# StoreyLab/terastructure

Hardware: AMD Instinct MI355X
Metric: SNP-minibatch updates/sec (N x K phi+accum) at N=1000000 K=8 (higher is better)
Workload: dtype f64

## Files before the change

### terastructure_amd/csrc/tsamd_hybrid_kernels.h

```cpp
#pragma once
#include "tsamd_resident_kernels.h"

namespace tsamd {


template <int KT>
__device__ __forceinline__ void hy_gamma_one(double (&gx)[KT], double (&wx)[KT], uint32_t nib, uint32_t &cn, const double *s_sb, const DevParams &p) {
  const double mom = (double)(nib & 3u), dad = (double)((nib >> 2) & 3u);
  const bool ok = (nib & 15u) != 0u;
  double s0 = 0.0, s1 = 0.0;
  uint32_t zo = 0u;
  asm volatile("" : "+v"(zo));
  const double *sbv = s_sb + zo;
#pragma unroll
  for (int k = 0; k < KT; ++k) {
    s0 = fma(wx[k], sbv[2 * k], s0);
    s1 = fma(wx[k], sbv[2 * k + 1], s1);
  }
  const double rho = ok ? fast_rsqrt(p.nodetau0 + (double)cn) : 0.0;
  const double inv = fast_rcp(s0 * s1) * (rho * p.gamma_scale);
  const double c0 = (mom * s1) * inv, c1 = (dad * s0) * inv, keep = 1.0 - rho, ra = rho * p.alpha;
#pragma unroll
  for (int k = 0; k < KT; ++k) gx[k] = fma(wx[k], fma(c0, sbv[2 * k], c1 * sbv[2 * k + 1]), fma(keep, gx[k], ra));
  if constexpr (KT <= 8) gamma_to_w<KT>(gx, wx); else gamma_to_w_lean<KT>(gx, wx);
  cn = ok ? cn + 1u : cn;
}

template <int KT, int WR, bool STREAM>
__global__ __launch_bounds__(256, 1) void ts_hybrid(Ctl *ctl_a, double *w_a, uint32_t npad_a, uint32_t chunk_a, uint32_t par_arg,
                                                    const uint32_t *sched, uint32_t n_sched, ResXchg *xb, uint32_t serial, const DevParams p) {
  constexpr int BLOCK = 256, kWaves = BLOCK / 64, R = hy_reg_items(KT), Q = hy_lds_items(KT), RQ = R + Q;
  constexpr bool BS = KT <= 12, BSC = KT <= 8;
  constexpr uint32_t J = 2 * KT;
  static_assert(resident_vec(KT) == 1 && R <= 16 && Q >= 1 && Q <= 16, "one individual per item; an item class's codes share one register");
  __shared__ __attribute__((aligned(16))) double s_eb[J];
  __shared__ __attribute__((aligned(16))) double s_sb[J];
  __shared__ double s_lam[J], s_diff[J], s_tot[res_tot_doubles<KT, WR>()], s_plam[J], s_peb[J];
  __shared__ double s_red[kWaves * J];
  __shared__ int s_alive[4];
  __shared__ double s_w[Q][KT][BLOCK];
  const uint32_t par = par_arg & 1u;
  Ctl *ctl = ctl_a;
  const State *S = &ctl->st[par ^ 1u];
  State *W = &ctl->st[par];
  const uint32_t svalid = S->valid, sloc = S->loc, shol = S->hol, siters = S->iters, sidx = S->idx;
  const unsigned long long epoch_now = S->epoch + 1ull;
  const uint32_t xseq0 = ctl->xseq;
  uint32_t tid = threadIdx.x;
  const size_t np = npad_a;
  const uint32_t nitems = npad_a;
  const uint32_t begin = blockIdx.x * chunk_a, end = min(begin + chunk_a, nitems);
  uint32_t i0 = begin + tid;
  uint32_t cnt = (i0 < end) ? (end - i0 + BLOCK - 1u) / BLOCK : 0u;
  auto fresh = [&]() { asm volatile("" : "+v"(tid), "+v"(i0), "+v"(cnt)); };
  auto item_or_last = [&](uint32_t t) { return min(i0, nitems - 1u) + min(t, max(cnt, 1u) - 1u) * BLOCK; };
  const uint32_t cnt_wg = begin < end ? (end - begin + BLOCK - 1u) / BLOCK : 0u;
  const uint32_t scnt_wg = (STREAM && cnt_wg > (uint32_t)RQ) ? cnt_wg - (uint32_t)RQ : 0u;
  const uint32_t g = blockIdx.x % (uint32_t)kResGroups, m = blockIdx.x / (uint32_t)kResGroups;

  if (__hip_atomic_load(&xb->abort_word, __ATOMIC_RELAXED, __HIP_MEMORY_SCOPE_AGENT) != 0ull) return;
  if (n_sched == 0u) {
    if (blockIdx.x == 0) carry_state(S, W, J);
    return;
  }
  if (tid < 4) s_alive[tid] = 1;
  __syncthreads();
  uint32_t xcount = 1u;
  if (!res_exchange<KT, WR>(xb, p, xseq0 + 1u, 1u, 0.0, g, m, gridDim.x, s_tot, s_alive, tid, fail_code(xseq0 + 1u, true, par, serial),
                            WR == 0 ? (unsigned long long)p.probe_ticks : kResWaitTicks))
    return;
  if constexpr (WR > 0) {
    xcount += 1u;
    if (!res_exchange<KT, WR>(xb, p, xseq0 + xcount, 1u, 0.0, g, m, gridDim.x, s_tot, s_alive, tid, fail_code(xseq0 + xcount, true, par, serial),
                              kResWaitTicks / 3ull))
      return;
  }
  double buf[R][KT];
#pragma unroll
  for (int t = 0; t < R; ++t) {
#pragma unroll
    for (int k = 0; k < KT; ++k) buf[t][k] = (w_a + (size_t)k * np)[item_or_last((uint32_t)t)];
    if (t & 1) __builtin_amdgcn_sched_barrier(0);
  }
#pragma unroll
  for (int q = 0; q < Q; ++q) {
    const uint32_t i = item_or_last((uint32_t)(R + q));
#pragma unroll
    for (int k = 0; k < KT; ++k) s_w[q][k][tid] = (w_a + (size_t)k * np)[i];
  }
  auto load_codes = [&](uint32_t loc_, auto first_c, auto n_c) -> uint2 {
    constexpr int FIRST = decltype(first_c)::value, N = decltype(n_c)::value;
    const uint32_t *col = reinterpret_cast<const uint32_t *>(p.bed + (size_t)loc_ * p.colstride);
    uint32_t word[N];
#pragma unroll
    for (int t = 0; t < N; ++t) word[t] = col[item_or_last((uint32_t)(FIRST + t)) / 16u];
    uint32_t out[2] = {0u, 0u};
#pragma unroll
    for (int t = 0; t < N; ++t) {
      const uint32_t i = item_or_last((uint32_t)(FIRST + t));
      const uint32_t c = (uint32_t)(FIRST + t) < cnt ? (word[t] >> (2u * (i % 16u))) & 3u : 1u;
      out[t / 8] |= code_nibble(c) << (4u * (uint32_t)(t % 8));
    }
    return make_uint2(out[0], out[1]);
  };
  using IC0 = std::integral_constant<int, 0>;
  using ICR = std::integral_constant<int, R>;
  using ICQ = std::integral_constant<int, Q>;
  uint2 pcodes = svalid ? load_codes(sloc, IC0{}, ICR{}) : make_uint2(0u, 0u), pcodes2 = svalid ? load_codes(sloc, ICR{}, ICQ{}) : make_uint2(0u, 0u);
  if (tid < J) {
    s_sb[tid] = S->eb[tid];
    s_plam[tid] = svalid ? p.lam[(size_t)sloc * J + tid] : 0.0;
    s_peb[tid] = svalid ? p.eb[(size_t)sloc * J + tid] : 0.0;
  }
  bool do_gamma = svalid != 0u && shol == 0u;
  bool prev_valid = svalid != 0u;
  uint32_t prev_loc = sloc, prev_hol = shol, prev_iters = siters;
  bool w_dirty = false;
  unsigned long long tp_run = ctl->total_passes;
  uint32_t last_it = ctl->last_iters;
  auto count_snp_deferred = [&](uint32_t its) {
    const uint32_t bin = min(its, (uint32_t)TSAMD_PASS_HIST_BINS - 1u);
    __hip_atomic_fetch_add(&ctl->pass_hist[bin], 1ull, __ATOMIC_RELAXED, __HIP_MEMORY_SCOPE_AGENT);
    tp_run += (unsigned long long)its;
    last_it = its;
  };
#ifdef TSAMD_SCHED_TIME
  unsigned long long tk_gamma = 0, tk_sweep = 0, tk_xchg = 0, tk_epi = 0, tk_fold = 0, tk_mark = wall_clock64();
  const unsigned long long tk_start = tk_mark;
#define TSAMD_HK(acc)                               \
  do {                                              \
    const unsigned long long now_ = wall_clock64(); \
    acc += now_ - tk_mark;                          \
    tk_mark = now_;                                 \
  } while (0)
#else
#define TSAMD_HK(acc) \
  do {                \
  } while (0)
#endif
  __syncthreads();

  uint32_t iters = 0u;
  double lam_old = 0.0, eb_used = 0.0;
  double b0[BS ? KT : 1], b1[BS ? KT : 1], acc0[KT], acc1[KT];
  bool complete = false;
  uint2 codes = make_uint2(0u, 0u), codes2 = make_uint2(0u, 0u);
  uint32_t loc = 0u, hol = 0u;
  const uint32_t *col = nullptr;

  auto begin_pass = [&]() {
    fresh();
    iters += 1u;
    lam_old = s_lam[tid < J ? tid : 0u];
    eb_used = s_eb[tid < J ? tid : 0u];
#pragma unroll
    for (int k = 0; k < KT; ++k) {
      if constexpr (BSC) {
        b0[k] = uniform_f64(s_eb[2 * k]);
        b1[k] = uniform_f64(s_eb[2 * k + 1]);
      } else if constexpr (BS) {
        b0[k] = s_eb[2 * k];
        b1[k] = s_eb[2 * k + 1];
      }
      acc0[k] = acc1[k] = 0.0;
    }
  };
  auto consume = [&](const double (&wcur)[KT], uint32_t nib) {
    uint32_t zo = 0u;
    if constexpr (!BS) asm volatile("" : "+v"(zo));
    res_consume_md<KT, BS>(wcur, (double)(nib & 3u), (double)(nib >> 2), b0, b1, reinterpret_cast<const double2 *>(s_eb) + zo, acc0, acc1);
  };
  auto load_streamed = [&](uint32_t s, double (&wv)[KT], uint32_t &word) {
    const uint32_t i = item_or_last((uint32_t)RQ + s);
#pragma unroll
    for (int k = 0; k < KT; ++k) wv[k] = (w_a + (size_t)k * np)[i];
    word = col[i / 16u];
  };
  auto streamed_code = [&](uint32_t s, uint32_t word) -> uint32_t {
    const uint32_t i = item_or_last((uint32_t)RQ + s);
    return code_nibble((uint32_t)RQ + s < cnt ? (word >> (2u * (i % 16u))) & 3u : 1u);
  };
  double sa[KT], sbuf[KT];
  uint32_t worda = 0u, wordb = 0u;
  auto request_first = [&]() { load_streamed(0u, sa, worda); };
  auto sweep = [&]() {
#pragma unroll
    for (int t = 0; t < R; ++t) {
      if ((uint32_t)t >= cnt_wg) continue;
      fresh();
      double wcur[KT];
#pragma unroll
      for (int k = 0; k < KT; ++k) wcur[k] = buf[t][k];
      consume(wcur, nibble_of(codes, t));
      __builtin_amdgcn_sched_barrier(0);
    }
#pragma unroll
    for (int q = 0; q < Q; ++q) {
      if ((uint32_t)(R + q) >= cnt_wg) continue;
      fresh();
      double wcur[KT];
#pragma unroll
      for (int k = 0; k < KT; ++k) wcur[k] = s_w[q][k][tid];
      consume(wcur, nibble_of(codes2, q));
      __builtin_amdgcn_sched_barrier(0);
    }
    for (uint32_t s = 0; STREAM && s < scnt_wg; s += 2u) {
      fresh();
      load_streamed(s + 1u, sbuf, wordb);
      __builtin_amdgcn_sched_barrier(0);
      consume(sa, streamed_code(s, worda));
      __builtin_amdgcn_sched_barrier(0);
      if (s + 1u >= scnt_wg) break;
      fresh();
      load_streamed(s + 2u, sa, worda);
      __builtin_amdgcn_sched_barrier(0);
      consume(sbuf, streamed_code(s + 1u, wordb));
      __builtin_amdgcn_sched_barrier(0);
    }
  };
  auto finish_pass = [&]() -> bool {
    fresh();
    res_fold<KT>(acc0, acc1, s_red, tid);
    __syncthreads();
    TSAMD_HK(tk_fold);
    double mine = 0.0;
    if (tid < J) {
      mine = s_red[tid];
#pragma unroll
      for (int wv = 1; wv < kWaves; ++wv) mine += s_red[wv * J + tid];
    }
    xcount += 1u;
    const uint32_t tag = xseq0 + xcount;
    const bool ahead = STREAM && iters < p.max_inner;
    auto overlap = [&]() {
      if constexpr (STREAM)
        if (ahead) request_first();
    };
    if (!res_exchange<KT, WR, kResOneLevelGrid, ResLay<KT>>(xb, p, tag, 1u, mine, g, m, gridDim.x, s_tot, s_alive, tid, fail_code(tag, false, par, serial),
                                                            kResWaitTicks, overlap))
      return false;
    TSAMD_HK(tk_xchg);
    if (tid < J) epilogue_values(p, res_total<KT, WR>(s_tot, tid), eb_used, lam_old, s_lam, s_eb, s_diff);
    __syncthreads();
    complete = epilogue_complete(p, iters, J, s_diff);
    TSAMD_HK(tk_epi);
    return true;
  };

  for (uint32_t idx = 0; idx < n_sched; ++idx) {
    const uint32_t ent = sched[idx];
    loc = ent & 0x7fffffffu;
    hol = ent >> 31;
    fresh();
    if (tid < J) {
      const bool local = prev_valid && loc == prev_loc;
      const double gl = __hip_atomic_load(&p.lam[(size_t)loc * J + tid], __ATOMIC_RELAXED, __HIP_MEMORY_SCOPE_AGENT);
      const double ge = __hip_atomic_load(&p.eb[(size_t)loc * J + tid], __ATOMIC_RELAXED, __HIP_MEMORY_SCOPE_AGENT);
      s_lam[tid] = local ? s_plam[tid] : gl;
      s_eb[tid] = local ? s_peb[tid] : ge;
    }
    codes = load_codes(loc, IC0{}, ICR{});
    codes2 = load_codes(loc, ICR{}, ICQ{});
    iters = 0u;
    if (do_gamma) {
      const uint32_t *pcol = reinterpret_cast<const uint32_t *>(p.bed + (size_t)prev_loc * p.colstride);
      double gs[KT];
      uint32_t cs = 0u;
      auto load_gamma = [&](uint32_t i, double (&gq)[KT], uint32_t &cq) {
#pragma unroll
        for (int k = 0; k < KT; ++k) gq[k] = (p.gam + (size_t)k * np)[i];
        cq = p.cnt[i];
      };
      auto store_gamma = [&](uint32_t i, const double (&gq)[KT], uint32_t cq) {
#pragma unroll
        for (int k = 0; k < KT; ++k) (p.gam + (size_t)k * np)[i] = gq[k];
        p.cnt[i] = cq;
      };
      load_gamma(item_or_last(0u), gs, cs);
#pragma unroll
      for (int t = 0; t < RQ; ++t) {
        if ((uint32_t)t >= cnt_wg) continue;
        fresh();
        const uint32_t i = item_or_last((uint32_t)t);
        double gv[KT];
        uint32_t cv = cs;
#pragma unroll
        for (int k = 0; k < KT; ++k) gv[k] = gs[k];
        if ((uint32_t)(t + 1) < cnt_wg && t + 1 < RQ) load_gamma(item_or_last((uint32_t)t + 1u), gs, cs);
        __builtin_amdgcn_sched_barrier(0);
        double wcur[KT];
        if (t < R) {
#pragma unroll
          for (int k = 0; k < KT; ++k) wcur[k] = buf[t < R ? t : 0][k];
        } else {
#pragma unroll
          for (int k = 0; k < KT; ++k) wcur[k] = s_w[t < R ? 0 : t - R][k][tid];
        }
        const uint32_t pcode = t < R ? nibble_of(pcodes, t < R ? t : 0) : nibble_of(pcodes2, t < R ? 0 : t - R);
        hy_gamma_one<KT>(gv, wcur, pcode, cv, s_sb, p);
        if ((uint32_t)t < cnt) store_gamma(i, gv, cv);
        if (t < R) {
#pragma unroll
          for (int k = 0; k < KT; ++k) buf[t < R ? t : 0][k] = wcur[k];
        } else {
#pragma unroll
          for (int k = 0; k < KT; ++k) s_w[t < R ? 0 : t - R][k][tid] = wcur[k];
        }
        __builtin_amdgcn_sched_barrier(0);
      }
      if (STREAM && scnt_wg > 0u) {
        double wsn[KT];
        uint32_t pwn = 0u;
        auto load_sitem = [&](uint32_t s) {
          const uint32_t i = item_or_last((uint32_t)RQ + s);
          load_gamma(i, gs, cs);
#pragma unroll
          for (int k = 0; k < KT; ++k) wsn[k] = (w_a + (size_t)k * np)[i];
          pwn = pcol[i / 16u];
        };
        load_sitem(0u);
        for (uint32_t s = 0; s < scnt_wg; ++s) {
          fresh();
          const uint32_t i = item_or_last((uint32_t)RQ + s);
          double gv[KT], wcur[KT];
          uint32_t cv = cs;
          const uint32_t pw = pwn;
#pragma unroll
          for (int k = 0; k < KT; ++k) {
            gv[k] = gs[k];
            wcur[k] = wsn[k];
          }
          load_sitem(min(s + 1u, scnt_wg - 1u));
          __builtin_amdgcn_sched_barrier(0);
          const uint32_t pcode = code_nibble((uint32_t)RQ + s < cnt ? (pw >> (2u * (i % 16u))) & 3u : 1u);
          hy_gamma_one<KT>(gv, wcur, pcode, cv, s_sb, p);
          if ((uint32_t)RQ + s < cnt) {
            store_gamma(i, gv, cv);
#pragma unroll
            for (int k = 0; k < KT; ++k) (w_a + (size_t)k * np)[i] = wcur[k];
          }
          __builtin_amdgcn_sched_barrier(0);
        }
      }
      w_dirty = true;
    }
    col = reinterpret_cast<const uint32_t *>(p.bed + (size_t)loc * p.colstride);
    if constexpr (STREAM) request_first();
    __syncthreads();
    TSAMD_HK(tk_gamma);
    complete = false;
    while (!complete) {
      begin_pass();
      sweep();
      TSAMD_HK(tk_sweep);
      if (!finish_pass()) return;
    }
    const double fin_lam = s_lam[tid < J ? tid : 0u], fin_eb = s_eb[tid < J ? tid : 0u];
    if (blockIdx.x == 0) {
      if (tid < J) {
        __hip_atomic_store(&p.lam[(size_t)loc * J + tid], fin_lam, __ATOMIC_RELAXED, __HIP_MEMORY_SCOPE_AGENT);
        __hip_atomic_store(&p.eb[(size_t)loc * J + tid], fin_eb, __ATOMIC_RELAXED, __HIP_MEMORY_SCOPE_AGENT);
      }
      if (tid == 0) count_snp_deferred(iters);
      asm volatile("s_waitcnt vmcnt(0)" ::: "memory");
    }
    __syncthreads();
    if (tid < J) {
      s_sb[tid] = eb_used;
      s_plam[tid] = fin_lam;
      s_peb[tid] = fin_eb;
    }
    pcodes = codes;
    pcodes2 = codes2;
    do_gamma = hol == 0u;
    prev_valid = true;
    prev_loc = loc;
    prev_hol = hol;
    prev_iters = iters;
    __syncthreads();
  }

  if (w_dirty) {
#pragma unroll
    for (int t = 0; t < RQ; ++t) {
      fresh();
      if ((uint32_t)t < cnt) {
        const uint32_t i = i0 + (uint32_t)t * BLOCK;
#pragma unroll
        for (int k = 0; k < KT; ++k) (w_a + (size_t)k * np)[i] = t < R ? buf[t < R ? t : 0][k] : s_w[t < R ? 0 : t - R][k][tid];
      }
    }
  }
  fresh();
  if (blockIdx.x == 0) {
    if (tid < J) {
      W->lam[tid] = s_plam[tid];
      W->eb[tid] = s_sb[tid];
    }
    if (tid == 0) {
      W->idx = sidx + n_sched;
      W->valid = 1u;
      W->loc = prev_loc;
      W->hol = prev_hol;
// ... 29 lines not shown
```

### terastructure_amd/csrc/tsamd_resident_kernels.h

```cpp
#pragma once
#include <type_traits>

#include "tsamd_kernels.h"

namespace tsamd {
#ifndef TSAMD_NOCOL_K
#define TSAMD_NOCOL_K 0
#endif
#ifndef TSAMD_GAMMA_SB_READLANE
#define TSAMD_GAMMA_SB_READLANE 1
#endif
#ifndef TSAMD_REPL_READLANE
#define TSAMD_REPL_READLANE 1
#endif


constexpr int res_blocks(int k) { return (4 * k + 31) / 32; }
constexpr int kResMaxGran = 32 * res_blocks(kResidentMaxK);
constexpr int kResRegionRows = kResGroups * kResMembers + 2 * kResGroups;
constexpr int kResWideGran = 512;
struct ResXchg {
  unsigned long long abort_word;
  unsigned long long pad_[31];
  unsigned long long gran[2 * kResRegionRows * kResMaxGran];
// ... 581 lines not shown
    for (int k = 0; k < KT; ++k) wv[k] = reinterpret_cast<const WT *>(w_a + (size_t)k * np)[i];
  };
  if (tid < 4) s_alive[tid] = 1;

  RowSum<BLOCK> rowsum;
  rowsum.issue(partials_a + (size_t)(par ^ 1u) * kMaxGrid * J, nrows_hint, J);
  const PendingIn pin = load_pending(S, J);
  WT buf[kItems][KT];
  load_rows(item_or_last(0), buf[0]);
  __builtin_amdgcn_sched_barrier(0);
  uint32_t codes = 0u;
  {
    const uint32_t *col = reinterpret_cast<const uint32_t *>(p.bed + (size_t)sloc * p.colstride);
    uint32_t word[kItems];
#pragma unroll
    for (int t = 0; t < kItems; ++t) word[t] = col[item_or_last((uint32_t)t) / RC::kItemsPerWord];
#pragma unroll
    for (int t = 0; t < kItems; ++t) {
      const uint32_t i = item_or_last((uint32_t)t);
      const uint32_t c = (uint32_t)t < cnt ? (word[t] >> (RC::kCodeBits * (i % RC::kItemsPerWord))) & RC::kMask : RC::kMissing;
      codes |= c << (RC::kCodeBits * (uint32_t)t);
    }
  }
  __builtin_amdgcn_sched_barrier(0);

  if (aborted != 0ull) return;
  const bool pending = svalid != 0u && sdone == 0u;
  const unsigned long long epoch_now = S->epoch + 1ull;
  if (!pending) {
    if (blockIdx.x == 0) carry_state(S, W, J);
    return;
  }
  const double vrow = (snrows == nrows_hint) ? rowsum.finish()
                                             : row_partial_sum<BLOCK>(partials_a + (size_t)(par ^ 1u) * kMaxGrid * J, snrows, J);
  bool complete = finish_pending<BLOCK>(p, pin, vrow, J, s_fin, s_lam, s_eb, s_diff);
  uint32_t iters = siters;
  double eb_used = pin.eb_used;
  const uint32_t g = blockIdx.x % (uint32_t)kResGroups, m = blockIdx.x / (uint32_t)kResGroups;
  double lam_old = 0.0;
  double b0[BS ? KT : 1], b1[BS ? KT : 1], acc0[KT], acc1[KT];
  auto begin_pass = [&]() {
    iters += 1u;
    lam_old = s_lam[tid < J ? tid : 0u];
    eb_used = s_eb[tid < J ? tid : 0u];
#pragma unroll
    for (int k = 0; k < KT; ++k) {
      if constexpr (BSC) {
        b0[k] = uniform_f64(s_eb[2 * k]);
        b1[k] = uniform_f64(s_eb[2 * k + 1]);
      } else if constexpr (BS) {
        b0[k] = s_eb[2 * k];
        b1[k] = s_eb[2 * k + 1];
      }
      acc0[k] = acc1[k] = 0.0;
    }
  };
  auto consume = [&](int t, const WT (&wv)[KT]) {
    uint32_t zo = 0u;
    if constexpr (!BS) asm volatile("" : "+v"(zo));
    res_consume<KT, VEC, BS>(wv, (codes >> (RC::kCodeBits * (uint32_t)t)) & RC::kMask, b0, b1, reinterpret_cast<const double2 *>(s_eb) + zo, acc0,
                             acc1);
  };
  uint32_t xcount = 0u;
  auto finish_pass = [&]() -> bool {
    res_fold<KT>(acc0, acc1, s_red, tid);
    __syncthreads();
    double row = 0.0;
    if (tid < J) {
      row = s_red[tid];
#pragma unroll
      for (int wv = 1; wv < kWaves; ++wv) row += s_red[wv * J + tid];
    }
    if (iters >= p.max_inner) {
      if (tid < J) (partials_a + (size_t)par * kMaxGrid * J)[(size_t)blockIdx.x * J + tid] = row;
      if (blockIdx.x == 0) {
        if (tid < J) {
          W->lam[tid] = lam_old;
          W->eb[tid] = eb_used;
        }
        if (tid == 0) {
          W->idx = sidx;
          W->valid = 1u;
          W->loc = sloc;
          W->hol = shol;
          W->iters = iters;
          W->done = 0u;
          W->nrows = gridDim.x;
          W->epoch = epoch_now;
          ctl->xseq = xseq0 + xcount;
        }
      }
      return true;
    }
    xcount += 1u;
    const uint32_t tag = xseq0 + xcount;
    if (!res_exchange<KT, 0, (KT <= 8 ? 16 : 0)>(xb, p, tag, 1u, row, g, m, gridDim.x, s_tot, s_alive, tid, fail_code(tag, xcount == 1u, par, serial),
                             xcount == 1u ? (unsigned long long)p.probe_ticks : kResWaitTicks))
      return true;
    if (tid < J) epilogue_values(p, s_tot[tid], eb_used, lam_old, s_lam, s_eb, s_diff);
    __syncthreads();
    complete = epilogue_complete(p, iters, J, s_diff);
    return false;
  };
  auto publish = [&]() {
    if (blockIdx.x == 0) {
      publish_complete_v(p, ctl, W, J, sidx, sloc, shol, iters, epoch_now, eb_used, s_lam, s_eb);
      if (tid == 0) ctl->xseq = xseq0 + xcount;
    }
  };

  if (complete) {
    publish();
    return;
  }
  begin_pass();
  if constexpr (kItems > 1) load_rows(item_or_last(1u), buf[1]);
#pragma unroll
  for (int t = 0; t < kItems; ++t) {
    if (t + 2 < kItems) load_rows(item_or_last((uint32_t)t + 2u), buf[t + 2]);
    __builtin_amdgcn_sched_barrier(0);
    consume(t, buf[t]);
    __builtin_amdgcn_sched_barrier(0);
  }
  if (finish_pass()) return;
  for (;;) {
    if (complete) {
      publish();
      return;
    }
    begin_pass();
#pragma unroll
    for (int t = 0; t < kItems; ++t) {
      consume(t, buf[t]);
      __builtin_amdgcn_sched_barrier(0);
    }
    if (finish_pass()) return;
  }
}

constexpr int sched_lds_items(int k, int items, int vec) {
#ifdef TSAMD_SCHED_LDS_ITEMS
  return TSAMD_SCHED_LDS_ITEMS < items ? TSAMD_SCHED_LDS_ITEMS : items;
#else
  const int small = 1536 + 26 * 2 * k * 8;
  const int per_item = (k * 8 + 4) * vec * 256, n = (160 * 1024 - small) / per_item;
  return n < items ? n : items;
#endif
}
constexpr int sched_next_streamed(int t, int lds, int items) {
  for (int u = t + 1; u < items; ++u)
    if (((u + 1) * lds) / items == (u * lds) / items) return u;
  return items;
}

template <int KT, bool PARTIAL, int WR>
__global__ __launch_bounds__(256, 1) void ts_schedule(Ctl *ctl_a, double *w_a, uint32_t npad_a, uint32_t chunk_a, uint32_t par_arg,
                                                      const uint32_t *sched, uint32_t n_sched, ResXchg *xb, uint32_t serial, const DevParams p) {
  constexpr int BLOCK = 256, kWaves = BLOCK / 64, VEC = resident_vec(KT), kItems = sched_items(KT, WR);
  constexpr bool BS = KT <= 24, BSC = KT <= 8;
  using LN = Lanes<VEC>;
  using WT = typename LN::T;
  using CT = typename LN::C;
  using RC = ResCodes<VEC>;
  constexpr uint32_t J = 2 * KT;
  static_assert(VEC == 1 && kItems <= 16, "one individual per item; the items' genotype nibbles are packed into two registers");
  __shared__ __attribute__((aligned(16))) double s_eb[J];
  __shared__ __attribute__((aligned(16))) double s_sb[J];
  __shared__ double s_lam[J], s_diff[J], s_tot[res_tot_doubles<KT, WR>()], s_plam[J], s_peb[J];
  __shared__ double s_drow[J], s_dlam[J], s_dolam[J], s_doeb[J], s_ddiff[J];
#if defined(TSAMD_SHARED_EPILOGUE)
  constexpr bool kRepl = false;
#else
  constexpr bool kRepl = KT <= 8;
#endif
  __shared__ __attribute__((aligned(16))) double s_ebw[kWaves][J];
  __shared__ double s_diffw[kWaves][J];
  __shared__ double s_red[kWaves * J];
  __shared__ int s_alive[4];
  constexpr int kLds = sched_lds_items(KT, kItems, VEC);
  __shared__ WT s_gam[kLds > 0 ? kLds : 1][KT][BLOCK];
  __shared__ CT s_cn[kLds > 0 ? kLds : 1][BLOCK];
  auto is_lds = [](int t) { return ((t + 1) * kLds) / kItems != (t * kLds) / kItems; };
  auto lds_slot = [](int t) { return (t * kLds) / kItems; };
  const uint32_t par = par_arg & 1u;
  Ctl *ctl = ctl_a;
  const State *S = &ctl->st[par ^ 1u];
  State *W = &ctl->st[par];
  const uint32_t svalid = S->valid, sloc = S->loc, shol = S->hol, siters = S->iters, sidx = S->idx;
  const unsigned long long epoch_now = S->epoch + 1ull;
  const uint32_t xseq0 = ctl->xseq;
  uint32_t tid = threadIdx.x;
  const size_t np = npad_a;
  const uint32_t nitems = npad_a / (uint32_t)VEC;
  const uint32_t begin = blockIdx.x * chunk_a, end = min(begin + chunk_a, nitems);
  uint32_t i0 = begin + tid;
  uint32_t cnt = (i0 < end) ? min((end - i0 + BLOCK - 1u) / BLOCK, (uint32_t)kItems) : 0u;
  auto fresh = [&]() { asm volatile("" : "+v"(tid), "+v"(i0), "+v"(cnt)); };
  auto item_or_last = [&](uint32_t t) { return min(i0, nitems - 1u) + min(t, max(cnt, 1u) - 1u) * BLOCK; };
  const uint32_t cnt_wg = !PARTIAL ? (uint32_t)kItems : begin < end ? min((end - begin + BLOCK - 1u) / BLOCK, (uint32_t)kItems) : 0u;
  const uint32_t g = blockIdx.x % (uint32_t)kResGroups, m = blockIdx.x / (uint32_t)kResGroups;

  if (__hip_atomic_load(&xb->abort_word, __ATOMIC_RELAXED, __HIP_MEMORY_SCOPE_AGENT) != 0ull) return;
  if (n_sched == 0u) {
    if (blockIdx.x == 0) carry_state(S, W, J);
    return;
  }
  if (tid < 4) s_alive[tid] = 1;
  __syncthreads();
  uint32_t xcount = 1u;
  if (!res_exchange<KT, WR>(xb, p, xseq0 + 1u, 1u, 0.0, g, m, gridDim.x, s_tot, s_alive, tid, fail_code(xseq0 + 1u, true, par, serial),
                            WR == 0 ? (unsigned long long)p.probe_ticks : kResWaitTicks))
    return;
  if constexpr (WR > 0) {
    xcount += 1u;
    if (p.xchg_test_delay != 0u) {
      const unsigned long long t0 = wall_clock64();
      while (wall_clock64() - t0 < (unsigned long long)p.xchg_test_delay) __builtin_amdgcn_s_sleep(8);
    }
    if (!res_exchange<KT, WR>(xb, p, xseq0 + xcount, 1u, 0.0, g, m, gridDim.x, s_tot, s_alive, tid, fail_code(xseq0 + xcount, true, par, serial),
                              kResWaitTicks / 3ull))
      return;
  }
  WT buf[kItems][KT];
#pragma unroll
  for (int t = 0; t < kItems; ++t) {
#pragma unroll
    for (int k = 0; k < KT; ++k) buf[t][k] = reinterpret_cast<const WT *>(w_a + (size_t)k * np)[item_or_last((uint32_t)t)];
    if (t & 1) __builtin_amdgcn_sched_barrier(0);
  }
#pragma unroll
  for (int t = 0; t < kItems; ++t)
    if (is_lds(t)) {
      const uint32_t i = item_or_last((uint32_t)t);
#pragma unroll
      for (int k = 0; k < KT; ++k) s_gam[lds_slot(t)][k][tid] = reinterpret_cast<const WT *>(p.gam + (size_t)k * np)[i];
      s_cn[lds_slot(t)][tid] = reinterpret_cast<const CT *>(p.cnt)[i];
    }
  auto get_item = [&](int t, WT (&wv)[KT]) {
#pragma unroll
    for (int k = 0; k < KT; ++k) wv[k] = buf[t][k];
  };
  auto put_item = [&](int t, const WT (&wv)[KT]) {
#pragma unroll
    for (int k = 0; k < KT; ++k) buf[t][k] = wv[k];
  };
  auto get_lgamma = [&](int t, WT (&gv)[KT], CT &cv) {
#pragma unroll
    for (int k = 0; k < KT; ++k) gv[k] = s_gam[lds_slot(t)][k][tid];
    cv = s_cn[lds_slot(t)][tid];
  };
  auto put_lgamma = [&](int t, const WT (&gv)[KT], const CT &cv) {
#pragma unroll
    for (int k = 0; k < KT; ++k) s_gam[lds_slot(t)][k][tid] = gv[k];
    s_cn[lds_slot(t)][tid] = cv;
  };
  auto load_words = [&](uint32_t loc_, auto &word) {
    const uint32_t *col = reinterpret_cast<const uint32_t *>(p.bed + (size_t)loc_ * p.colstride);
#pragma unroll
    for (int t = 0; t < kItems; ++t) word[t] = col[item_or_last((uint32_t)t) / RC::kItemsPerWord];
  };
  auto pack_codes = [&](const auto &word) -> uint2 {
    uint32_t out[2] = {0u, 0u};
#pragma unroll
    for (int t = 0; t < kItems; ++t) {
      const uint32_t i = item_or_last((uint32_t)t);
      const uint32_t c = (uint32_t)t < cnt ? (word[t] >> (RC::kCodeBits * (i % RC::kItemsPerWord))) & RC::kMask : RC::kMissing;
      out[t / 8] |= code_nibble(c) << (4u * (uint32_t)(t % 8));
    }
    return make_uint2(out[0], out[1]);
  };
  auto load_codes = [&](uint32_t loc_) -> uint2 {
    uint32_t word[kItems];
    load_words(loc_, word);
    return pack_codes(word);
  };
  uint2 pcodes = svalid ? load_codes(sloc) : make_uint2(0u, 0u);
  const double sb_state = S->eb[(tid & 63u) < J ? (tid & 63u) : 0u];
  if (tid < J) {
    s_sb[tid] = S->eb[tid];
    s_plam[tid] = svalid ? p.lam[(size_t)sloc * J + tid] : 0.0;
    s_peb[tid] = svalid ? p.eb[(size_t)sloc * J + tid] : 0.0;
  }
  bool do_gamma = svalid != 0u && shol == 0u;
  bool prev_valid = svalid != 0u;
  uint32_t prev_loc = sloc, prev_hol = shol, prev_iters = siters;
  bool w_dirty = false;
  bool deferred = false;
  uint32_t dloc = 0u, diters = 0u;
  bool pub_pending = false;
  unsigned long long tp_run = ctl->total_passes;
  uint32_t last_it = ctl->last_iters;
  auto count_snp_deferred = [&](uint32_t its) {
    const uint32_t bin = min(its, (uint32_t)TSAMD_PASS_HIST_BINS - 1u);
    __hip_atomic_fetch_add(&ctl->pass_hist[bin], 1ull, __ATOMIC_RELAXED, __HIP_MEMORY_SCOPE_AGENT);
    tp_run += (unsigned long long)its;
    last_it = its;
  };
#ifdef TSAMD_SCHED_RAMP
  unsigned long long ramp_mark = wall_clock64();
  uint32_t ramp_idx = 0u;
#endif
#ifdef TSAMD_SCHED_TIME
  unsigned long long tk_gamma = 0, tk_first = 0, tk_rest = 0, tk_xchg = 0, tk_head = 0, tk_tail = 0, tk_mark = wall_clock64();
  unsigned long long tk_fold = 0, tk_epi = 0, tk_sweep = 0;
  const unsigned long long tk_start = tk_mark;
#define TSAMD_TK(acc)                         \
  do {                                        \
    const unsigned long long now_ = wall_clock64(); \
    acc += now_ - tk_mark;                    \
    tk_mark = now_;                           \
  } while (0)
#else
#define TSAMD_TK(acc) \
  do {                \
  } while (0)
#endif
  __syncthreads();

  uint32_t iters = 0u;
  double lam_old = 0.0, eb_used = 0.0;
  double b0[BS ? KT : 1], b1[BS ? KT : 1], acc0[KT], acc1[KT];
  bool complete = false;
  constexpr bool kColAhead = !(KT == 16 || KT == 14 || (KT == 24 && WR == 8)) && KT != TSAMD_NOCOL_K;
  uint2 codes = kColAhead ? load_codes(sched[0] & 0x7fffffffu) : make_uint2(0u, 0u);
  uint32_t nword[kColAhead ? kItems : 1];
  double eb_ran = sb_state;
  auto begin_pass = [&]() {
    fresh();
    iters += 1u;
    const double *bsrc = kRepl ? s_ebw[tid >> 6] : s_eb;
    if constexpr (kRepl) {
      eb_ran = eb_used;
    } else {
      lam_old = s_lam[tid < J ? tid : 0u];
      eb_used = s_eb[tid < J ? tid : 0u];
    }
#pragma unroll
    for (int k = 0; k < KT; ++k) {
      if constexpr (kRepl && BSC && TSAMD_REPL_READLANE) {
        b0[k] = lane_f64(eb_used, 2 * k);
        b1[k] = lane_f64(eb_used, 2 * k + 1);
      } else if constexpr (BSC) {
        b0[k] = uniform_f64(bsrc[2 * k]);
        b1[k] = uniform_f64(bsrc[2 * k + 1]);
      } else if constexpr (BS) {
        b0[k] = bsrc[2 * k];
        b1[k] = bsrc[2 * k + 1];
      }
      acc0[k] = acc1[k] = 0.0;
    }
  };
  auto sweep = [&]() {
#ifdef TSAMD_SCHED_TIME
    const unsigned long long ts0 = wall_clock64();
#endif
#pragma unroll
    for (int t = 0; t < kItems; ++t) {
      if (PARTIAL && (uint32_t)t >= cnt_wg) continue;
      fresh();
      WT wcur[KT];
      get_item(t, wcur);
      uint32_t zo = 0u;
      if constexpr (!BS) asm volatile("" : "+v"(zo));
      const double2 *bl = reinterpret_cast<const double2 *>(kRepl ? s_ebw[tid >> 6] : s_eb) + zo;
      {
        const uint32_t nib = nibble_of(codes, t);
        res_consume_md<KT, BS>(wcur, (double)(nib & 3u), (double)(nib >> 2), b0, b1, bl, acc0, acc1);
      }
      __builtin_amdgcn_sched_barrier(0);
    }
#ifdef TSAMD_SCHED_TIME
    tk_sweep += wall_clock64() - ts0;
#endif
  };
  auto finish_pass = [&](bool defer) -> bool {
    fresh();
#ifdef TSAMD_SCHED_TIME
    const unsigned long long tf0 = wall_clock64();
#endif
    if (kRepl && pub_pending) {
      asm volatile("s_waitcnt vmcnt(0)" ::: "memory");
      pub_pending = false;
    }
    res_fold<KT>(acc0, acc1, s_red, tid);
    __syncthreads();
#ifdef TSAMD_SCHED_TIME
    const unsigned long long tx0 = wall_clock64();
    tk_fold += tx0 - tf0;
#endif
    double mine = 0.0;
    if (tid < J) {
      mine = s_red[tid];
#pragma unroll
      for (int wv = 1; wv < kWaves; ++wv) mine += s_red[wv * J + tid];
    }
    if (defer) {
      if (tid < J) s_drow[tid] = mine;
      if (tid < J) s_dlam[tid] = lam_old;
      complete = true;
      return true;
    }
    const uint32_t width = deferred ? 2u : 1u;
    if (deferred && tid >= 64u && tid < 64u + J) mine = s_drow[tid - 64u];
    if (!kRepl && pub_pending) {
      asm volatile("s_waitcnt vmcnt(0)" ::: "memory");
      pub_pending = false;
    }
    xcount += 1u;
    const uint32_t tag = xseq0 + xcount;
    if (!res_exchange<KT, WR>(xb, p, tag, width, mine, g, m, gridDim.x, s_tot, s_alive, tid, fail_code(tag, false, par, serial), kResWaitTicks))
      return false;
#ifdef TSAMD_SCHED_TIME
    const unsigned long long te0 = wall_clock64();
    tk_xchg += te0 - tx0;
#endif
    if constexpr (kRepl) {
      const uint32_t lane = tid & 63u, wave = tid >> 6;
      if (lane < J) {
        double nw, ebn, df;
        epilogue_values_reg(p, lane, res_total<KT, WR>(s_tot, lane), eb_used, lam_old, nw, ebn, df);
        lam_old = nw;
        eb_used = ebn;
        if constexpr (!(BSC && TSAMD_REPL_READLANE)) s_ebw[wave][lane] = ebn;
        s_diffw[wave][lane] = df;
      }
      if (deferred) {
        if (blockIdx.x == 0) {
          if (wave == 1u && lane < J) {
            double nw, ebn, df;
            epilogue_values_reg(p, lane, res_total<KT, WR>(s_tot, J + lane), s_sb[lane], s_dlam[lane], nw, ebn, df);
            __hip_atomic_store(&p.lam[(size_t)dloc * J + lane], nw, __ATOMIC_RELAXED, __HIP_MEMORY_SCOPE_AGENT);
            __hip_atomic_store(&p.eb[(size_t)dloc * J + lane], ebn, __ATOMIC_RELAXED, __HIP_MEMORY_SCOPE_AGENT);
          }
          if (tid == 0) count_snp_deferred(diters);
          pub_pending = true;
        }
        deferred = false;
      }
      complete = epilogue_complete(p, iters, J, s_diffw[wave]);
    } else {
    if (tid < J) epilogue_values(p, res_total<KT, WR>(s_tot, tid), eb_used, lam_old, s_lam, s_eb, s_diff);
    if (deferred && blockIdx.x == 0 && tid >= 64u && tid < 64u + J)
      epilogue_values_at(p, tid - 64u, res_total<KT, WR>(s_tot, J + tid - 64u), s_sb[tid - 64u], s_dlam[tid - 64u], s_dolam, s_doeb, s_ddiff);
    __syncthreads();
    if (deferred) {
      if (blockIdx.x == 0) {
        if (tid < J) {
          __hip_atomic_store(&p.lam[(size_t)dloc * J + tid], s_dolam[tid], __ATOMIC_RELAXED, __HIP_MEMORY_SCOPE_AGENT);
          __hip_atomic_store(&p.eb[(size_t)dloc * J + tid], s_doeb[tid], __ATOMIC_RELAXED, __HIP_MEMORY_SCOPE_AGENT);
        }
        if (tid == 0) count_snp_deferred(diters);
        pub_pending = true;
      }
      deferred = false;
    }
    if constexpr (KT > 8) complete = epilogue_complete_wave<J>(p, iters, s_diff, tid & 63u); else complete = epilogue_complete(p, iters, J, s_diff);
    }
#ifdef TSAMD_SCHED_TIME
    tk_epi += wall_clock64() - te0;
#endif
    return true;
  };

  uint32_t loc = 0, hol = 0;
  uint32_t ent_n = sched[0], ent_nn = sched[min(1u, n_sched - 1u)];
  double nlam = 0.0, neb = 0.0;
  if (tid < J) {
    nlam = p.lam[(size_t)(ent_n & 0x7fffffffu) * J + tid];
    neb = p.eb[(size_t)(ent_n & 0x7fffffffu) * J + tid];
  }
  for (uint32_t idx = 0; idx < n_sched; ++idx) {
    const uint32_t ent = ent_n;
    loc = ent & 0x7fffffffu;
    hol = ent >> 31;
    ent_n = ent_nn;
    ent_nn = sched[min(idx + 2u, n_sched - 1u)];
    if (tid < J) {
      const bool local = prev_valid && loc == prev_loc;
      s_lam[tid] = local ? s_plam[tid] : nlam;
      s_eb[tid] = local ? s_peb[tid] : neb;
    }
    fresh();
    if constexpr (!kColAhead) codes = load_codes(loc);
    __syncthreads();
    if constexpr (kRepl) {
      const uint32_t lane = tid & 63u, wave = tid >> 6;
      lam_old = s_lam[lane < J ? lane : 0u];
      eb_used = s_eb[lane < J ? lane : 0u];
      if constexpr (!(BSC && TSAMD_REPL_READLANE))
        if (lane < J) s_ebw[wave][lane] = eb_used;
    }
    iters = 0u;
    TSAMD_TK(tk_head);
    if (do_gamma) {
      WT gs[KT];
      CT cs;
      auto load_gamma = [&](uint32_t i, WT (&gq)[KT], CT &cq) {
#pragma unroll
        for (int k = 0; k < KT; ++k) gq[k] = reinterpret_cast<const WT *>(p.gam + (size_t)k * np)[i];
        cq = reinterpret_cast<const CT *>(p.cnt)[i];
      };
#if defined(TSAMD_LITERAL_STEP)
      constexpr bool kLeanStep = false;
#elif defined(TSAMD_LEAN_STEP)
      constexpr bool kLeanStep = true;
#else
      constexpr bool kLeanStep = PARTIAL || KT > 8;
#endif
      constexpr bool kSbScalar = kRepl && BSC && TSAMD_GAMMA_SB_READLANE != 0;
      double sbs[kSbScalar ? J : 1];
      if constexpr (kSbScalar) {
#pragma unroll
        for (int j = 0; j < (int)J; ++j) sbs[j] = lane_f64(eb_ran, j);
      }
      auto gamma_one = [&](double (&gx)[KT], double (&wx)[KT], uint32_t nib, uint32_t &cn) {
        const double mom = (double)(nib & 3u), dad = (double)((nib >> 2) & 3u);
        const bool ok = (nib & 15u) != 0u;
        double s0 = 0.0, s1 = 0.0;
        uint32_t zo = 0u;
        asm volatile("" : "+v"(zo));
        const double *sbv = s_sb + zo;
        auto sb = [&](int j) -> double {
          if constexpr (kSbScalar) return sbs[j]; else return sbv[j];
        };
#pragma unroll
        for (int k = 0; k < KT; ++k) {
          s0 = fma(wx[k], sb(2 * k), s0);
          s1 = fma(wx[k], sb(2 * k + 1), s1);
        }
        const double rho = ok ? fast_rsqrt(p.nodetau0 + (double)cn) : 0.0;
        if constexpr (kLeanStep) {
          const double inv = fast_rcp(s0 * s1) * (rho * p.gamma_scale);
          const double c0 = (mom * s1) * inv, c1 = (dad * s0) * inv, keep = 1.0 - rho, ra = rho * p.alpha;
#pragma unroll
          for (int k = 0; k < KT; ++k) gx[k] = fma(wx[k], fma(c0, sb(2 * k), c1 * sb(2 * k + 1)), fma(keep, gx[k], ra));
        } else {
          const double c0 = mom * fast_rcp(s0), c1 = dad * fast_rcp(s1);
#pragma unroll
          for (int k = 0; k < KT; ++k) {
            const double e = c0 * (wx[k] * sb(2 * k)) + c1 * (wx[k] * sb(2 * k + 1));
            gx[k] += rho * (p.alpha + p.gamma_scale * e - gx[k]);
          }
        }
        if constexpr (KT <= 8) gamma_to_w<KT>(gx, wx); else gamma_to_w_lean<KT>(gx, wx);
        cn = ok ? cn + 1u : cn;
      };
      constexpr int kFirstStreamed = sched_next_streamed(-1, kLds, kItems);
      if (kFirstStreamed < kItems) load_gamma(item_or_last((uint32_t)kFirstStreamed), gs, cs);
#pragma unroll
      for (int t = 0; t < kItems; ++t) {
        if (PARTIAL && (uint32_t)t >= cnt_wg) continue;
        fresh();
        const uint32_t i = item_or_last((uint32_t)t);
        const bool mine = (uint32_t)t < cnt;
        WT gv[KT];
        CT cv;
        if (is_lds(t)) {
          get_lgamma(t, gv, cv);
        } else {
#pragma unroll
          for (int k = 0; k < KT; ++k) gv[k] = gs[k];
          cv = cs;
          constexpr int kNone = kItems;
          const int nxt = sched_next_streamed(t, kLds, kItems);
          if (nxt < kNone) load_gamma(item_or_last((uint32_t)nxt), gs, cs);
        }
        __builtin_amdgcn_sched_barrier(0);
        WT wcur[KT];
        get_item(t, wcur);
        uint32_t pcode = nibble_of(pcodes, t);
        if constexpr (VEC == 2) {
#pragma unroll 1
          for (int v = 0; v < 2; ++v) {
            double gx[KT], wx[KT];
#pragma unroll
            for (int k = 0; k < KT; ++k) {
              gx[k] = gv[k].x;
              wx[k] = wcur[k].x;
            }
            uint32_t cn = cv.x;
            gamma_one(gx, wx, pcode, cn);
            pcode >>= 2;
            cv.x = cv.y;
            cv.y = cn;
#pragma unroll
            for (int k = 0; k < KT; ++k) {
              gv[k].x = gv[k].y;
              gv[k].y = gx[k];
              wcur[k].x = wcur[k].y;
              wcur[k].y = wx[k];
            }
          }
        } else {
          gamma_one(gv, wcur, pcode, cv);
        }
        if (is_lds(t)) {
          put_lgamma(t, gv, cv);
        } else if (mine) {
#pragma unroll
          for (int k = 0; k < KT; ++k) reinterpret_cast<WT *>(p.gam + (size_t)k * np)[i] = gv[k];
          reinterpret_cast<CT *>(p.cnt)[i] = cv;
        }
        put_item(t, wcur);
        __builtin_amdgcn_sched_barrier(0);
      }
      w_dirty = true;
    }
    TSAMD_TK(tk_gamma);
    begin_pass();
    sweep();
    if (!finish_pass(false)) return;
    TSAMD_TK(tk_first);
    fresh();
    if (tid < J) {
      nlam = __hip_atomic_load(&p.lam[(size_t)(ent_n & 0x7fffffffu) * J + tid], __ATOMIC_RELAXED, __HIP_MEMORY_SCOPE_AGENT);
      neb = __hip_atomic_load(&p.eb[(size_t)(ent_n & 0x7fffffffu) * J + tid], __ATOMIC_RELAXED, __HIP_MEMORY_SCOPE_AGENT);
    }
    if constexpr (kColAhead) load_words(ent_n & 0x7fffffffu, nword);
    while (!complete) {
      begin_pass();
      sweep();
#ifdef TSAMD_NO_DEFER
      const bool defer = false;
#else
      const bool defer = iters >= p.max_inner && idx + 1u < n_sched && (ent_n & 0x7fffffffu) != loc &&
                         (idx + 2u >= n_sched || (ent_nn & 0x7fffffffu) != loc);
#endif
      if (!finish_pass(defer)) return;
      if (defer) {
        deferred = true;
        dloc = loc;
        diters = iters;
      }
    }
    TSAMD_TK(tk_rest);
    const double fin_lam = kRepl ? lam_old : s_lam[tid < J ? tid : 0u], fin_eb = kRepl ? eb_used : s_eb[tid < J ? tid : 0u];
    if (!deferred && blockIdx.x == 0) {
      if (tid < J) {
        __hip_atomic_store(&p.lam[(size_t)loc * J + tid], fin_lam, __ATOMIC_RELAXED, __HIP_MEMORY_SCOPE_AGENT);
        __hip_atomic_store(&p.eb[(size_t)loc * J + tid], fin_eb, __ATOMIC_RELAXED, __HIP_MEMORY_SCOPE_AGENT);
      }
      if (tid == 0) count_snp_deferred(iters);
      asm volatile("s_waitcnt vmcnt(0)" ::: "memory");
    }
    __syncthreads();
    if (tid < J) s_sb[tid] = kRepl ? eb_ran : eb_used;
    if (tid < J) {
      s_plam[tid] = fin_lam;
      s_peb[tid] = fin_eb;
    }
    pcodes = codes;
    fresh();
    if constexpr (kColAhead) codes = pack_codes(nword);
    do_gamma = hol == 0u;
    prev_valid = true;
    prev_loc = loc;
    prev_hol = hol;
    prev_iters = iters;
    __syncthreads();
    TSAMD_TK(tk_tail);
#ifdef TSAMD_SCHED_RAMP
    if (blockIdx.x == 0 && tid == 0) {
      const uint32_t marks[8] = {5u, 20u, 50u, 100u, 200u, 500u, 1000u, 2000u};
      for (int q = 0; q < 8; ++q)
        if (idx + 1u == marks[q]) {
          const unsigned long long now = wall_clock64();
          printf("ts_schedule ramp: SNPs up to %u: %.2f us per SNP in this range (launch of %u)\n", marks[q],
                 (now - ramp_mark) * 0.01 / (double)(marks[q] - ramp_idx), n_sched);
          ramp_mark = now;
          ramp_idx = marks[q];
        }
    }
#endif
  }

  if (w_dirty) {
#pragma unroll
    for (int t = 0; t < kItems; ++t) {
      fresh();
      if ((uint32_t)t < cnt) {
        const uint32_t i = i0 + (uint32_t)t * BLOCK;
        WT wcur[KT];
        get_item(t, wcur);
#pragma unroll
        for (int k = 0; k < KT; ++k) reinterpret_cast<WT *>(w_a + (size_t)k * np)[i] = wcur[k];
        if (is_lds(t)) {
          WT gv[KT];
          CT cv;
          get_lgamma(t, gv, cv);
#pragma unroll
          for (int k = 0; k < KT; ++k) reinterpret_cast<WT *>(p.gam + (size_t)k * np)[i] = gv[k];
          reinterpret_cast<CT *>(p.cnt)[i] = cv;
        }
      }
    }
  }
  fresh();
  if (blockIdx.x == 0) {
    if (tid < J) {
      W->lam[tid] = s_plam[tid];
      W->eb[tid] = s_sb[tid];
    }
    if (tid == 0) {
      W->idx = sidx + n_sched;
      W->valid = 1u;
      W->loc = prev_loc;
      W->hol = prev_hol;
      W->iters = prev_iters;
      W->done = 1u;
      W->nrows = 0u;
      W->epoch = epoch_now;
      ctl->xseq = xseq0 + xcount;
      ctl->total_passes = tp_run;
      ctl->last_iters = last_it;
      if (p.host_error) {
        __hip_atomic_store(p.host_error + 1, (unsigned long long)last_it, __ATOMIC_RELAXED, __HIP_MEMORY_SCOPE_SYSTEM);
        __hip_atomic_store(p.host_error + 2, tp_run, __ATOMIC_RELAXED, __HIP_MEMORY_SCOPE_SYSTEM);
      }
      asm volatile("s_waitcnt vmcnt(0)" ::: "memory");
#ifdef TSAMD_SCHED_TIME
      if (n_sched >= 16u)
        printf("ts_schedule n=%u exchanges=%u | per SNP (us): head %.2f gamma %.2f first pass %.2f later passes %.2f tail %.2f | "
               "in exchanges %.2f, in folds %.2f, in epilogues %.2f, in sweeps %.2f | whole launch %.1f us\n", n_sched, xcount, tk_head * 0.01 / n_sched,
               tk_gamma * 0.01 / n_sched, tk_first * 0.01 / n_sched, tk_rest * 0.01 / n_sched, tk_tail * 0.01 / n_sched, tk_xchg * 0.01 / n_sched,
               tk_fold * 0.01 / n_sched, tk_epi * 0.01 / n_sched, tk_sweep * 0.01 / n_sched, (wall_clock64() - tk_start) * 0.01);
#endif
    }
    __syncthreads();
    if (p.host_error && tid < (uint32_t)TSAMD_PASS_HIST_BINS)
      __hip_atomic_store(p.host_error + 3 + tid, __hip_atomic_load(&ctl->pass_hist[tid], __ATOMIC_RELAXED, __HIP_MEMORY_SCOPE_AGENT),
                         __ATOMIC_RELAXED, __HIP_MEMORY_SCOPE_SYSTEM);
  }
#undef TSAMD_TK
}

}
```

Baseline: 13760.

## Stage schedule entries in an LDS ring prefetched during exchange waits

Replaces per-iteration global reads of the SNP schedule with a double-buffered 16-entry LDS ring. The next block is fetched by a few threads inside the exchange overlap hook, so the load latency hides behind the grid-wide wait. It also batches the initial LDS fills of w/gamma through registers so those loads are issued together rather than serialized. This adds LDS use, extra ring-indexing logic and a dependence on the ring being filled before entries are read, a risk if the refill timing is wrong.

```diff
diff --git a/terastructure_amd/csrc/tsamd_hybrid_kernels.h b/terastructure_amd/csrc/tsamd_hybrid_kernels.h
--- a/terastructure_amd/csrc/tsamd_hybrid_kernels.h
+++ b/terastructure_amd/csrc/tsamd_hybrid_kernels.h
@@ -39,6 +39,7 @@
   __shared__ double s_red[kWaves * J];
   __shared__ int s_alive[4];
   __shared__ double s_w[Q][KT][BLOCK];
+  __shared__ SchedRing s_sched;
   const uint32_t par = par_arg & 1u;
   Ctl *ctl = ctl_a;
   const State *S = &ctl->st[par ^ 1u];
@@ -75,18 +76,38 @@
                               kResWaitTicks / 3ull))
       return;
   }
+  uint32_t ring_first = 0u;
+  if (tid < 2u * kSchedBlock) ring_first = sched_ring_request(sched, tid, n_sched);
+  {
+    constexpr int kFillBatch = 48 / KT > 5 ? 5 : 48 / KT < 1 ? 1 : 48 / KT;
+#pragma unroll
+    for (int q0 = 0; q0 < Q; q0 += kFillBatch) {
+      double fw[kFillBatch][KT];
+#pragma unroll
+      for (int u = 0; u < kFillBatch; ++u)
+        if (q0 + u < Q) {
+          const uint32_t i = item_or_last((uint32_t)(R + q0 + u));
+#pragma unroll
+          for (int k = 0; k < KT; ++k) fw[u][k] = (w_a + (size_t)k * np)[i];
+        }
+      __builtin_amdgcn_sched_barrier(0);
+#pragma unroll
+      for (int u = 0; u < kFillBatch; ++u)
+        if (q0 + u < Q) {
+#pragma unroll
+          for (int k = 0; k < KT; ++k) s_w[q0 + u][k][tid] = fw[u][k];
+        }
+      __builtin_amdgcn_sched_barrier(0);
+    }
+  }
+  if (tid < 2u * kSchedBlock) s_sched[tid / kSchedBlock][tid % kSchedBlock] = ring_first;
+  __builtin_amdgcn_sched_barrier(0);
   double buf[R][KT];
 #pragma unroll
   for (int t = 0; t < R; ++t) {
 #pragma unroll
     for (int k = 0; k < KT; ++k) buf[t][k] = (w_a + (size_t)k * np)[item_or_last((uint32_t)t)];
     if (t & 1) __builtin_amdgcn_sched_barrier(0);
-  }
-#pragma unroll
-  for (int q = 0; q < Q; ++q) {
-    const uint32_t i = item_or_last((uint32_t)(R + q));
-#pragma unroll
-    for (int k = 0; k < KT; ++k) s_w[q][k][tid] = (w_a + (size_t)k * np)[i];
   }
   auto load_codes = [&](uint32_t loc_, auto first_c, auto n_c) -> uint2 {
     constexpr int FIRST = decltype(first_c)::value, N = decltype(n_c)::value;
@@ -146,6 +167,8 @@
   bool complete = false;
   uint2 codes = make_uint2(0u, 0u), codes2 = make_uint2(0u, 0u);
   uint32_t loc = 0u, hol = 0u;
+  bool ring_fetch = false;
+  uint32_t ring_at = 0u;
   const uint32_t *col = nullptr;
 
   auto begin_pass = [&]() {
@@ -233,12 +256,14 @@
     const uint32_t tag = xseq0 + xcount;
     const bool ahead = STREAM && iters < p.max_inner;
     auto overlap = [&]() {
+      if (ring_fetch && tid < kSchedBlock) s_sched[(ring_at / kSchedBlock) & 1u][tid] = sched_ring_request(sched, ring_at + tid, n_sched);
       if constexpr (STREAM)
         if (ahead) request_first();
     };
     if (!res_exchange<KT, WR, kResOneLevelGrid, ResLay<KT>>(xb, p, tag, 1u, mine, g, m, gridDim.x, s_tot, s_alive, tid, fail_code(tag, false, par, serial),
                                                             kResWaitTicks, overlap))
       return false;
+    ring_fetch = false;
     TSAMD_HK(tk_xchg);
     if (tid < J) epilogue_values(p, res_total<KT, WR>(s_tot, tid), eb_used, lam_old, s_lam, s_eb, s_diff);
     __syncthreads();
@@ -248,7 +273,9 @@
   };
 
   for (uint32_t idx = 0; idx < n_sched; ++idx) {
-    const uint32_t ent = sched[idx];
+    const uint32_t ent = sched_ring_entry(s_sched, idx, n_sched);
+    ring_fetch = sched_ring_fetches(idx, n_sched);
+    ring_at = idx + kSchedBlock;
     loc = ent & 0x7fffffffu;
     hol = ent >> 31;
     fresh();
diff --git a/terastructure_amd/csrc/tsamd_resident_kernels.h b/terastructure_amd/csrc/tsamd_resident_kernels.h
--- a/terastructure_amd/csrc/tsamd_resident_kernels.h
+++ b/terastructure_amd/csrc/tsamd_resident_kernels.h
@@ -757,6 +757,24 @@
     if (((u + 1) * lds) / items == (u * lds) / items) return u;
   return items;
 }
+constexpr int sched_lds_item(int slot, int lds, int items) {
+  for (int u = 0; u < items; ++u)
+    if (((u + 1) * lds) / items != (u * lds) / items && (u * lds) / items == slot) return u;
+  return items;
+}
+
+constexpr uint32_t kSchedBlock = 16u;
+using SchedRing = uint32_t[2][kSchedBlock];
+__device__ __forceinline__ uint32_t sched_ring_entry(const SchedRing &ring, uint32_t idx, uint32_t n) {
+  const uint32_t i = min(idx, n - 1u);
+  return ring[(i / kSchedBlock) & 1u][i % kSchedBlock];
+}
+__device__ __forceinline__ bool sched_ring_fetches(uint32_t idx, uint32_t n) {
+  return idx != 0u && idx % kSchedBlock == 0u && idx + kSchedBlock < n;
+}
+__device__ __forceinline__ uint32_t sched_ring_request(const uint32_t *sched, uint32_t i, uint32_t n) {
+  return __hip_atomic_load(&sched[min(i, n - 1u)], __ATOMIC_RELAXED, __HIP_MEMORY_SCOPE_SYSTEM);
+}
 
 template <int KT, bool PARTIAL, int WR>
 __global__ __launch_bounds__(256, 1) void ts_schedule(Ctl *ctl_a, double *w_a, uint32_t npad_a, uint32_t chunk_a, uint32_t par_arg,
@@ -785,6 +803,7 @@
   constexpr int kLds = sched_lds_items(KT, kItems, VEC);
   __shared__ WT s_gam[kLds > 0 ? kLds : 1][KT][BLOCK];
   __shared__ CT s_cn[kLds > 0 ? kLds : 1][BLOCK];
+  __shared__ SchedRing s_sched;
   auto is_lds = [](int t) { return ((t + 1) * kLds) / kItems != (t * kLds) / kItems; };
   auto lds_slot = [](int t) { return (t * kLds) / kItems; };
   const uint32_t par = par_arg & 1u;
@@ -826,6 +845,36 @@
                               kResWaitTicks / 3ull))
       return;
   }
+  uint32_t ring_first = 0u;
+  if (tid < 2u * kSchedBlock) ring_first = sched_ring_request(sched, tid, n_sched);
+  constexpr bool kFillFirst = !(KT == 21 || KT == 24);
+  if constexpr (kFillFirst) {
+    constexpr int kFillBatch = 48 / (KT + 1) > 5 ? 5 : 48 / (KT + 1) < 1 ? 1 : 48 / (KT + 1);
+#pragma unroll
+    for (int s0 = 0; s0 < kLds; s0 += kFillBatch) {
+      WT fg[kFillBatch][KT];
+      CT fc[kFillBatch];
+#pragma unroll
+      for (int u = 0; u < kFillBatch; ++u)
+        if (s0 + u < kLds) {
+          const uint32_t i = item_or_last((uint32_t)sched_lds_item(s0 + u, kLds, kItems));
+#pragma unroll
+          for (int k = 0; k < KT; ++k) fg[u][k] = reinterpret_cast<const WT *>(p.gam + (size_t)k * np)[i];
+          fc[u] = reinterpret_cast<const CT *>(p.cnt)[i];
+        }
+      __builtin_amdgcn_sched_barrier(0);
+#pragma unroll
+      for (int u = 0; u < kFillBatch; ++u)
+        if (s0 + u < kLds) {
+#pragma unroll
+          for (int k = 0; k < KT; ++k) s_gam[s0 + u][k][tid] = fg[u][k];
+          s_cn[s0 + u][tid] = fc[u];
+        }
+      __builtin_amdgcn_sched_barrier(0);
+    }
+  }
+  if (tid < 2u * kSchedBlock) s_sched[tid / kSchedBlock][tid % kSchedBlock] = ring_first;
+  __builtin_amdgcn_sched_barrier(0);
   WT buf[kItems][KT];
 #pragma unroll
   for (int t = 0; t < kItems; ++t) {
@@ -833,14 +882,16 @@
     for (int k = 0; k < KT; ++k) buf[t][k] = reinterpret_cast<const WT *>(w_a + (size_t)k * np)[item_or_last((uint32_t)t)];
     if (t & 1) __builtin_amdgcn_sched_barrier(0);
   }
-#pragma unroll
-  for (int t = 0; t < kItems; ++t)
-    if (is_lds(t)) {
-      const uint32_t i = item_or_last((uint32_t)t);
-#pragma unroll
-      for (int k = 0; k < KT; ++k) s_gam[lds_slot(t)][k][tid] = reinterpret_cast<const WT *>(p.gam + (size_t)k * np)[i];
-      s_cn[lds_slot(t)][tid] = reinterpret_cast<const CT *>(p.cnt)[i];
-    }
+  if constexpr (!kFillFirst) {
+#pragma unroll
+    for (int t = 0; t < kItems; ++t)
+      if (is_lds(t)) {
+        const uint32_t i = item_or_last((uint32_t)t);
+#pragma unroll
+        for (int k = 0; k < KT; ++k) s_gam[lds_slot(t)][k][tid] = reinterpret_cast<const WT *>(p.gam + (size_t)k * np)[i];
+        s_cn[lds_slot(t)][tid] = reinterpret_cast<const CT *>(p.cnt)[i];
+      }
+  }
   auto get_item = [&](int t, WT (&wv)[KT]) {
 #pragma unroll
     for (int k = 0; k < KT; ++k) wv[k] = buf[t][k];
@@ -927,7 +978,7 @@
   double b0[BS ? KT : 1], b1[BS ? KT : 1], acc0[KT], acc1[KT];
   bool complete = false;
   constexpr bool kColAhead = !(KT == 16 || KT == 14 || (KT == 24 && WR == 8)) && KT != TSAMD_NOCOL_K;
-  uint2 codes = kColAhead ? load_codes(sched[0] & 0x7fffffffu) : make_uint2(0u, 0u);
+  uint2 codes = kColAhead ? load_codes(sched_ring_entry(s_sched, 0u, n_sched) & 0x7fffffffu) : make_uint2(0u, 0u);
   uint32_t nword[kColAhead ? kItems : 1];
   double eb_ran = sb_state;
   auto begin_pass = [&]() {
@@ -978,7 +1029,7 @@
     tk_sweep += wall_clock64() - ts0;
 #endif
   };
-  auto finish_pass = [&](bool defer) -> bool {
+  auto finish_pass = [&](bool defer, auto overlap) -> bool {
     fresh();
 #ifdef TSAMD_SCHED_TIME
     const unsigned long long tf0 = wall_clock64();
@@ -1013,7 +1064,8 @@
     }
     xcount += 1u;
     const uint32_t tag = xseq0 + xcount;
-    if (!res_exchange<KT, WR>(xb, p, tag, width, mine, g, m, gridDim.x, s_tot, s_alive, tid, fail_code(tag, false, par, serial), kResWaitTicks))
+    if (!res_exchange<KT, WR>(xb, p, tag, width, mine, g, m, gridDim.x, s_tot, s_alive, tid, fail_code(tag, false, par, serial), kResWaitTicks,
+                              overlap))
       return false;
 #ifdef TSAMD_SCHED_TIME
     const unsigned long long te0 = wall_clock64();
@@ -1068,7 +1120,7 @@
   };
 
   uint32_t loc = 0, hol = 0;
-  uint32_t ent_n = sched[0], ent_nn = sched[min(1u, n_sched - 1u)];
+  uint32_t ent_n = sched_ring_entry(s_sched, 0u, n_sched), ent_nn = sched_ring_entry(s_sched, 1u, n_sched);
   double nlam = 0.0, neb = 0.0;
   if (tid < J) {
     nlam = p.lam[(size_t)(ent_n & 0x7fffffffu) * J + tid];
@@ -1079,7 +1131,7 @@
     loc = ent & 0x7fffffffu;
     hol = ent >> 31;
     ent_n = ent_nn;
-    ent_nn = sched[min(idx + 2u, n_sched - 1u)];
+    ent_nn = sched_ring_entry(s_sched, idx + 2u, n_sched);
     if (tid < J) {
       const bool local = prev_valid && loc == prev_loc;
       s_lam[tid] = local ? s_plam[tid] : nlam;
@@ -1214,7 +1266,11 @@
     TSAMD_TK(tk_gamma);
     begin_pass();
     sweep();
-    if (!finish_pass(false)) return;
+    if (!finish_pass(false, [&]() {
+          if (sched_ring_fetches(idx, n_sched) && tid < kSchedBlock)
+            s_sched[(idx / kSchedBlock + 1u) & 1u][tid] = sched_ring_request(sched, idx + kSchedBlock + tid, n_sched);
+        }))
+      return;
     TSAMD_TK(tk_first);
     fresh();
     if (tid < J) {
@@ -1231,7 +1287,7 @@
       const bool defer = iters >= p.max_inner && idx + 1u < n_sched && (ent_n & 0x7fffffffu) != loc &&
                          (idx + 2u >= n_sched || (ent_nn & 0x7fffffffu) != loc);
 #endif
-      if (!finish_pass(defer)) return;
+      if (!finish_pass(defer, NoOverlap())) return;
       if (defer) {
         deferred = true;
         dloc = loc;
```

Measured after the change: 13870, median of 6. No clear change (+0.8%).
